# knowhunger/go-libp2p-pubsub

Hardware: AMD Instinct MI355X
Metric: peer-topic score updates/s + msg deliveries/s @1M peers, 1-8 GPUs, %HBM BW (higher is better)
Workload: dtype f64; 1 GPU; cfg3: 1M peers x 8 topics, full P1-P7 refreshScores()+score() per DecayInterval, connectSome d=6 overlay, spam-test topic params; peers_per_gpu=1000000, topics=8, pairs_per_gpu=11999954, records_per_gpu=95999632, parallelism=observers range-sharded, 1 shard(s), no exchange

## Files before the change

### go-libp2p-pubsub_amd/csrc/gsx_device.h

```cpp
#pragma once

#include <hip/hip_runtime.h>
#include <stdint.h>

namespace gsx {

struct DevTopicParams {
    double topic_weight;
    double w1, cap1;
    int64_t q1;
    double inv_q1;
    double w2, d2, cap2;
    double w3, d3, cap3, thr3;
    int64_t win3, act3;
    double w3b, d3b;
    double w4, d4;
    int32_t scored;
    int32_t pad;
};

__host__ __device__ __forceinline__ double q1_inverse(int64_t q1) { return q1 > 0 ? 1.0 / (double)q1 : 0.0; }

struct DevPeerParams {
    double topic_score_cap;
    double w5;
    double w6;
    int64_t thr6;
    double w7, thr7, d7;
    double decay_to_zero;
    int64_t retain_ns;
};

constexpr int KARG_TOPICS = 8;
struct KernParams {
    DevPeerParams pp;
    DevTopicParams tp[KARG_TOPICS];
};

constexpr int TILE = 64;
constexpr int NFIELD = 5;
enum Field { FMD = 0, MMD = 1, MFP = 2, IMD = 3, GRAFT = 4 };

__host__ __device__ __forceinline__ size_t rec_index(uint64_t p, uint32_t t, uint32_t n_topics, int field) {
    return (((p / TILE) * n_topics + t) * NFIELD + field) * TILE + (p % TILE);
}
__host__ __device__ __forceinline__ size_t flag_index(uint64_t p, uint32_t t, uint32_t n_topics) {
    return ((p / TILE) * n_topics + t) * TILE + (p % TILE);
}

constexpr uint8_t ZM_ZERO = 0, ZM_MAYBE = 1;
__host__ __device__ __forceinline__ size_t zmap_index(uint64_t p, uint32_t t, uint32_t n_topics, int field) {
    return ((p / TILE) * n_topics + t) * 2 + (size_t)(field - MFP);
}
__host__ __device__ __forceinline__ size_t zmap_bytes(uint64_t n_tiles, uint32_t n_topics) {
    return ((n_tiles * n_topics * 2 + 3) / 4 + 1) * 4;
}

constexpr int PZ_APP = 0, PZ_P6 = 1, PZ_ENTRY = 4;
__host__ __device__ __forceinline__ size_t pzmap_bytes(uint64_t n_tiles) { return (n_tiles + 1) * PZ_ENTRY; }

struct DevState {
    double* rec;
    uint8_t* rflags;
    uint8_t* zmap;
    uint8_t* pzmap;
    uint8_t* pflags;
    int64_t* expire;
    double* bp;
    double* app;
    const uint32_t* ipg;
    uint32_t* ipcount;
    double* score;
    const DevTopicParams* tp;
    uint64_t n_pairs;
    uint32_t n_topics;
    int64_t last_refresh;
    uint32_t phase;
    uint32_t wb_period;
    double decay_to_zero;
    double d7;
};

constexpr uint8_t REC_IN_MESH = 0x01;
constexpr uint8_t REC_ACTIVE = 0x02;
constexpr uint8_t REC_FRESH = 0x04;
constexpr uint8_t REC_EPOCH = 0x18;
constexpr int REC_EPOCH_SHIFT = 3;
constexpr uint8_t PAIR_PRESENT = 0x01;
constexpr uint8_t PAIR_CONNECTED = 0x02;
constexpr uint8_t PAIR_EPOCH = 0x0C;
constexpr int PAIR_EPOCH_SHIFT = 2;
constexpr uint32_t IPG_NONE = 0xFFFFFFFFu;
constexpr uint32_t IPG_WL = 0x80000000u;

struct DevEvent {
    uint32_t kind;
    uint32_t topic;
    uint64_t pair;
    int64_t now_ns;
    int64_t arg;
};

struct DevSynthSpec {
    uint64_t seed;
    int64_t now;
    double fmd_max, mmd_max, mfp_max, imd_max;
    double p_in_mesh;
    int64_t graft_window;
    double bp_max, p_disc, p_abs;
    int64_t expire_jitter;
    uint32_t sybil_first;
};

constexpr uint8_t EDGE_OUTBOUND = 0x01, EDGE_DIRECT = 0x02, EDGE_GOSSIPSUB = 0x04, EDGE_FLOODSUB = 0x08,
                  EDGE_NO_PX = 0x10;
constexpr uint32_t ROUTER_FLOODSUB = 0, ROUTER_GOSSIPSUB = 1, ROUTER_RANDOMSUB = 2;
constexpr uint32_t NO_PAIR = 0xFFFFFFFFu;
constexpr uint8_t FWD_FORWARD = 0x01;
constexpr uint8_t FWD_PUBLISH = 0x02;
constexpr uint8_t FWD_RSUB_CAND = 0x04;
constexpr uint8_t FWD_SEND = 0x07;
constexpr uint8_t FWD_GIN = 0x08;
constexpr int RANDOMSUB_D = 6;
// ... 814 lines not shown
```

### go-libp2p-pubsub_amd/csrc/gsx_engine.cpp

```cpp
#include <hip/hip_runtime.h>

#include <algorithm>
#include <map>
#include <atomic>
#include <chrono>
#include <array>
#include <cmath>
#include <cstdio>
#include <cstdlib>
#include <cstring>
#include <deque>
#include <functional>
#include <string>
#include <unordered_map>
#include <unordered_set>
#include <vector>

#include "../../include/gsx.h"
#include "gsx_device.h"

namespace {

constexpr int64_t kSecond = 1000000000LL;
constexpr int64_t kTimeCacheDuration = 120 * kSecond;
constexpr uint64_t kHostScoreMax = 1u << 16;

bool invalid_number(double x) { return std::isnan(x) || std::isinf(x); }

enum { kDeliveryUnknown = 0, kDeliveryValid, kDeliveryInvalid, kDeliveryIgnored, kDeliveryThrottled };

struct RecKey {
    uint32_t obs;
    uint64_t msg;
    bool operator==(const RecKey& o) const { return obs == o.obs && msg == o.msg; }
};
struct RecKeyHash {
    size_t operator()(const RecKey& k) const {
        uint64_t x = k.msg ^ (uint64_t(k.obs) * 0x9E3779B97F4A7C15ULL);
        x ^= x >> 31;
        x *= 0xbf58476d1ce4e5b9ULL;
        x ^= x >> 29;
        return size_t(x);
    }
};
struct DeliveryRecord {
    int status = kDeliveryUnknown;
    int64_t first_seen = 0;
    int64_t validated = 0;
    bool validated_set = false;
    std::vector<uint64_t> peers;
    bool peers_nil = false;
};

}

struct gsx_engine {
    int device = 0;
    hipStream_t stream = nullptr;
    hipEvent_t ev_start = nullptr, ev_stop = nullptr, ev_staged = nullptr;
    std::string err;

    uint32_t T = 0;
    gsx_peer_score_params pp{};
    bool pp_set = false;
    gsx_thresholds th{};
    gsx_topic_score_params tp[GSX_MAX_TOPICS]{};
    bool scored[GSX_MAX_TOPICS]{};
    gsx::DevTopicParams* d_tp = nullptr;

    bool loaded = false;
    uint32_t n_nodes = 0;
    uint64_t E = 0, rs = 0, n_tiles = 0;
    int64_t last_refresh = 0;
    uint32_t phase = 0;
    uint32_t wb_period = 4;
    bool retained_possible = false;
    int64_t retain_horizon = INT64_MIN;
    uint64_t purge_launches = 0;
    std::vector<int64_t> row_ptr;
    std::vector<int32_t> col_host;
    std::vector<uint32_t> pair_obs;
    std::vector<uint32_t> ipg_host;
    std::vector<uint32_t> group_ip;
    std::vector<uint8_t> ip_wl;
    uint32_t n_groups = 0;

    double* d_rec = nullptr;
    uint8_t* d_rflags = nullptr;
    uint8_t* d_zmap = nullptr;
    uint8_t* d_pzmap = nullptr;
    void* d_tmp = nullptr;
    uint32_t* d_nbad = nullptr;
    uint8_t *d_pflags = nullptr, *d_eflags = nullptr;
    int64_t* d_expire = nullptr;
    double *d_bp = nullptr, *d_app = nullptr, *d_score = nullptr;
    uint32_t *d_ipg = nullptr, *d_ipcount = nullptr;
    int32_t* d_col = nullptr;
    int64_t* d_row_ptr = nullptr;
    uint32_t* d_rev = nullptr;
    std::vector<uint8_t> eflags_host;
    bool floodsub_peers = true;
    int64_t max_deg = 0;

    gsx_gossipsub_params gp{};
    int64_t* d_backoff = nullptr;
    uint8_t* d_bo8 = nullptr;
    uint64_t *d_ctl = nullptr, *d_resp = nullptr;
    uint8_t* d_dirty = nullptr;
// ... 549 lines not shown
}

gsx::DevTopicParams dev_topic_params(const gsx_engine* e, uint32_t t);

gsx::KernParams kern_params(const gsx_engine* e) {
    gsx::KernParams k{};
    k.pp = dev_peer_params(e);
    for (uint32_t t = 0; t < e->T && t < (uint32_t)gsx::KARG_TOPICS; ++t) k.tp[t] = dev_topic_params(e, t);
    return k;
}

gsx::DevTopicParams dev_topic_params(const gsx_engine* e, uint32_t t) {
    gsx::DevTopicParams d{};
    const gsx_topic_score_params& p = e->tp[t];
    d.topic_weight = p.topic_weight;
    d.w1 = p.time_in_mesh_weight;
    d.cap1 = p.time_in_mesh_cap;
    d.q1 = e->scored[t] ? p.time_in_mesh_quantum_ns : 1;
    d.inv_q1 = gsx::q1_inverse(d.q1);
    d.w2 = p.first_message_deliveries_weight;
    d.d2 = p.first_message_deliveries_decay;
    d.cap2 = p.first_message_deliveries_cap;
    d.w3 = p.mesh_message_deliveries_weight;
    d.d3 = p.mesh_message_deliveries_decay;
    d.cap3 = p.mesh_message_deliveries_cap;
    d.thr3 = p.mesh_message_deliveries_threshold;
    d.win3 = p.mesh_message_deliveries_window_ns;
    d.act3 = p.mesh_message_deliveries_activation_ns;
    d.w3b = p.mesh_failure_penalty_weight;
    d.d3b = p.mesh_failure_penalty_decay;
    d.w4 = p.invalid_message_deliveries_weight;
    d.d4 = p.invalid_message_deliveries_decay;
    d.scored = e->scored[t] ? 1 : 0;
    return d;
}

int upload_topic_params(gsx_engine* e) {
    gsx::DevTopicParams h[GSX_MAX_TOPICS]{};
    for (uint32_t t = 0; t < e->T; ++t) h[t] = dev_topic_params(e, t);
    HIPCHK(e, hipMemcpyAsync(e->d_tp, h, sizeof(gsx::DevTopicParams) * GSX_MAX_TOPICS, hipMemcpyHostToDevice,
                             e->stream));
    HIPCHK(e, hipStreamSynchronize(e->stream));
    return GSX_OK;
}

void seen_release(gsx_engine* e, uint64_t* p, size_t ) {
    if (!p) return;
    auto it = e->seen_cap.find(p);
    e->seen_pool.emplace_back(it != e->seen_cap.end() ? it->second : 0, p);
}
uint64_t* seen_acquire(gsx_engine* e, size_t words) {
    size_t best = e->seen_pool.size();
    for (size_t i = 0; i < e->seen_pool.size(); ++i)
        if (e->seen_pool[i].first >= words && (best == e->seen_pool.size() || e->seen_pool[i].first < e->seen_pool[best].first))
            best = i;
    if (best < e->seen_pool.size()) {
        uint64_t* p = e->seen_pool[best].second;
        e->seen_pool.erase(e->seen_pool.begin() + (long)best);
        return p;
    }
    constexpr size_t kSlab = 4, kSlabMaxBytes = 64ull << 20;
    const size_t w = (std::max<size_t>(words, 1) + 31) & ~(size_t)31;
    const size_t n = 8 * w <= kSlabMaxBytes ? kSlab : 1;
    uint64_t* p = nullptr;
    if (hipMalloc((void**)&p, 8 * w * n) != hipSuccess) {
        if (n == 1 || hipMalloc((void**)&p, 8 * w) != hipSuccess) return nullptr;
// ... 1497 lines not shown
    return GSX_OK;
}

int gsx_refresh(gsx_engine* e, int64_t now) {
    if (!e) return GSX_EINVAL;
    if (!e->loaded) return fail(e, GSX_ESTATE, "no overlay loaded");
    if (int rc = fold_deferred(e)) return rc;
    int rc = flush(e);
    if (rc) return rc;
    const gsx::DevState s = dev_state(e);
    if (e->retained_possible) {
        HIPCHK(e, gsx::launch_purge(s, now, e->stream));
        ++e->purge_launches;
        if (now > e->retain_horizon) {
            e->retained_possible = false;
            e->retain_horizon = INT64_MIN;
        }
    }
    const bool region = e->t_active && e->t_used < e->t_max;
    HIPCHK(e, hipEventRecord(region ? e->tev[2 * e->t_used] : e->ev_start, e->stream));
    HIPCHK(e, rescore_all(e, s, now, true));
    HIPCHK(e, hipEventRecord(region ? e->tev[2 * e->t_used + 1] : e->ev_stop, e->stream));
    if (region) ++e->t_used;
    e->timed = !region;
    e->scores_exact();
    e->state_changed();
    e->last_refresh = now;
    e->phase = e->phase + 1 >= e->wb_period ? 0 : e->phase + 1;
    return GSX_OK;
}

int gsx_set_decay_writeback(gsx_engine* e, uint32_t k) {
    if (!e) return GSX_EINVAL;
    if (k != 1 && k != 2 && k != 4) return fail(e, GSX_EINVAL, "decay write-back period must be 1, 2 or 4");
    if (int rc = gx_busy(e)) return rc;
    if (int rc = fold_deferred(e)) return rc;
    if (int rc = flush(e)) return rc;
    if (int rc = materialize_all(e)) return rc;
    e->wb_period = k;
    return GSX_OK;
}

int gsx_last_refresh_ms(gsx_engine* e, float* ms) {
    if (!e || !ms) return GSX_EINVAL;
    if (!e->timed) return fail(e, GSX_ESTATE, "no refresh timed yet");
    HIPCHK(e, hipEventSynchronize(e->ev_stop));
    HIPCHK(e, hipEventElapsedTime(ms, e->ev_start, e->ev_stop));
    return GSX_OK;
}

int gsx_timing_begin(gsx_engine* e, uint32_t max_launches) {
    if (!e || max_launches == 0) return GSX_EINVAL;
    while (e->tev.size() < 2 * (size_t)max_launches) {
        hipEvent_t ev;
        HIPCHK(e, hipEventCreate(&ev));
        e->tev.push_back(ev);
    }
    e->t_max = max_launches;
    e->t_used = 0;
    e->t_active = true;
    return GSX_OK;
}

int gsx_timing_end(gsx_engine* e, double* total_ms, double* min_ms, double* max_ms, uint32_t* n) {
    if (!e || !total_ms || !n) return GSX_EINVAL;
    if (!e->t_active) return fail(e, GSX_ESTATE, "gsx_timing_begin not called");
    e->t_active = false;
    double sum = 0, lo = 0, hi = 0;
    for (uint32_t i = 0; i < e->t_used; ++i) {
        HIPCHK(e, hipEventSynchronize(e->tev[2 * i + 1]));
        float ms = 0;
        HIPCHK(e, hipEventElapsedTime(&ms, e->tev[2 * i], e->tev[2 * i + 1]));
// ... 5309 lines not shown
```

### go-libp2p-pubsub_amd/csrc/gsx_kernels.hip

```cpp
#include "gsx_ops.h"

namespace gsx {



template <int TT, bool REFRESH>
__global__ __launch_bounds__(256) void k_refresh_score(DevState s, KernParams kp, int64_t now,
                                                       const uint8_t* __restrict__ only,
                                                       const uint8_t* __restrict__ only2,
                                                       const unsigned long long* __restrict__ gate) {
    const uint64_t p = (uint64_t)blockIdx.x * 256u + threadIdx.x;
    if (p >= s.n_pairs) return;
    if (!REFRESH && gate && gate[0] + gate[1] == 0) return;
    if (!REFRESH && only && (!only[p] || (only2 && !only2[p]))) return;
    const int T = TT > 0 ? TT : (int)s.n_topics;
    const uint64_t lane = p % TILE;
    const uint64_t wtile = wave_uniform(p / TILE);
    const uint64_t zoff = wtile * (uint64_t)T * 2;
    uint32_t zm[TT > 0 ? TT : 1];
    if constexpr (TT > 0) {
#pragma unroll
        for (int t = 0; t < TT; ++t) zm[t] = zmap_pair(s.zmap, zoff + 2 * t);
    }
    const uint32_t pz = __builtin_amdgcn_readfirstlane(reinterpret_cast<const uint32_t*>(s.pzmap)[wtile]);
    const bool app_maybe = (pz >> (8 * PZ_APP)) & 0xFFu;
    const bool p6_maybe = !REFRESH || ((pz >> (8 * PZ_P6)) & 0xFFu);
    const uint8_t st = s.pflags[p];
    if (!(st & PAIR_PRESENT)) {
        s.score[p] = 0.0;
        return;
    }
    const DevPeerParams& pp = kp.pp;
    double p5 = 0.0;
    if (app_maybe) p5 = s.app[p];
    const bool conn = REFRESH && (st & PAIR_CONNECTED);
    const uint32_t phase = s.phase;
    const bool wb = REFRESH && phase + 1 >= s.wb_period;
    const bool lag = st & PAIR_CONNECTED;
    const uint8_t keep_conn = (uint8_t)~(REC_FRESH | (wb ? REC_EPOCH : 0));
    double* const tile = s.rec + (p / TILE) * (uint64_t)T * (NFIELD * TILE) + lane;
    uint8_t* const ftile = s.rflags + (p / TILE) * (uint64_t)T * TILE + lane;
    double score = 0.0;
    auto topic_step = [&](int t, const DevTopicParams& tp, double fmd, double mmd, double mfp, double imd,
                          int64_t graft, uint8_t fl, uint32_t zmt) {
        double* const r = tile + (uint64_t)t * (NFIELD * TILE);
        const double fmd0 = fmd, mmd0 = mmd, mfp0 = mfp, imd0 = imd;
        const uint32_t nd = (lag ? (phase - ((uint32_t)fl >> REC_EPOCH_SHIFT)) & 3u : 0u) + (conn ? 1u : 0u);
        const uint32_t nd0 = __builtin_amdgcn_readfirstlane(nd);
        auto decay_all = [&]() {
            fmd = decay(fmd, tp.d2, pp.decay_to_zero);
            mmd = decay(mmd, tp.d3, pp.decay_to_zero);
            mfp = decay(mfp, tp.d3b, pp.decay_to_zero);
            imd = decay(imd, tp.d4, pp.decay_to_zero);
        };
        if (__ballot(nd != nd0) == 0) {
            for (uint32_t i = 0; i < nd0; ++i) decay_all();
        } else {
            for (uint32_t i = 0; i < nd; ++i) decay_all();
        }
        if (wb) {
            if (conn && __double_as_longlong(fmd) != __double_as_longlong(fmd0)) __builtin_nontemporal_store(fmd, r + FMD * TILE);
            if (conn && __double_as_longlong(mmd) != __double_as_longlong(mmd0)) __builtin_nontemporal_store(mmd, r + MMD * TILE);
            if (conn && __double_as_longlong(mfp) != __double_as_longlong(mfp0)) __builtin_nontemporal_store(mfp, r + MFP * TILE);
            if (conn && __double_as_longlong(imd) != __double_as_longlong(imd0)) __builtin_nontemporal_store(imd, r + IMD * TILE);
        }
        const bool in_mesh = fl & REC_IN_MESH;
        int64_t mt = 0;
        if (conn) {
            mt = in_mesh ? now - graft : 0;
            const uint8_t nf = (uint8_t)((fl & keep_conn) | ((in_mesh && mt > tp.act3) ? REC_ACTIVE : 0));
            if (nf != fl) ftile[t * TILE] = nf;
            fl = nf;
        } else if (in_mesh && !(fl & REC_FRESH)) {
            mt = s.last_refresh - graft;
        }
        if constexpr (REFRESH) {
            if (zmt && __ballot(1) == ~0ull) {
                uint8_t* const zb = s.zmap + zoff + 2 * t;
                const bool z3 = (zmt & ZM_MFP_BITS) && __ballot(__double_as_longlong(mfp) != 0) == 0;
                const bool z4 = (zmt & ZM_IMD_BITS) && __ballot(__double_as_longlong(imd) != 0) == 0;
                if (z3 && !wb && __double_as_longlong(mfp0) != 0) r[MFP * TILE] = 0.0;
                if (z4 && !wb && __double_as_longlong(imd0) != 0) r[IMD * TILE] = 0.0;
                if (z3 && lane == 0) zb[0] = ZM_ZERO;
                if (z4 && lane == 0) zb[1] = ZM_ZERO;
            }
        }
        score += topic_score(tp, fl, mt, fmd, mmd, mfp, imd);
    };
    if constexpr (TT > 0) {
        double fmd[TT], mmd[TT], mfp[TT], imd[TT];
        int64_t gr[TT];
// ... 2 lines not shown
        for (int t = 0; t < TT; ++t) {
            if (!kp.tp[t].scored) continue;
            const double* const r = tile + (uint64_t)t * (NFIELD * TILE);
            fmd[t] = __builtin_nontemporal_load(r + FMD * TILE);
            mmd[t] = __builtin_nontemporal_load(r + MMD * TILE);
            mfp[t] = (zm[t] & ZM_MFP_BITS) ? __builtin_nontemporal_load(r + MFP * TILE) : 0.0;
            imd[t] = (zm[t] & ZM_IMD_BITS) ? __builtin_nontemporal_load(r + IMD * TILE) : 0.0;
            fl[t] = ftile[t * TILE];
            gr[t] = (TT > 1 || (fl[t] & REC_IN_MESH))
                        ? __builtin_nontemporal_load(reinterpret_cast<const int64_t*>(r) + GRAFT * TILE)
                        : 0;
        }
#pragma unroll
        for (int t = 0; t < TT; ++t) {
            if (!kp.tp[t].scored) continue;
            topic_step(t, kp.tp[t], fmd[t], mmd[t], mfp[t], imd[t], gr[t], fl[t], zm[t]);
        }
    } else {
        for (int t = 0; t < T; ++t) {
            const DevTopicParams& tp = s.tp[t];
            if (!tp.scored) continue;
            const double* const r = tile + (uint64_t)t * (NFIELD * TILE);
            const uint32_t zmt = zmap_pair(s.zmap, zoff + 2 * t);
            const uint8_t fl = ftile[t * TILE];
            const int64_t graft = (fl & REC_IN_MESH) ? reinterpret_cast<const int64_t*>(r)[GRAFT * TILE] : 0;
            const double fmd = __builtin_nontemporal_load(r + FMD * TILE), mmd = __builtin_nontemporal_load(r + MMD * TILE);
            const double mfp = (zmt & ZM_MFP_BITS) ? __builtin_nontemporal_load(r + MFP * TILE) : 0.0;
            const double imd = (zmt & ZM_IMD_BITS) ? __builtin_nontemporal_load(r + IMD * TILE) : 0.0;
            topic_step(t, tp, fmd, mmd, mfp, imd, graft, fl, zmt);
        }
    }
    const double bp0 = s.bp[p];
    double bp = bp0;
    const uint32_t nb = (lag ? (phase - ((uint32_t)st >> PAIR_EPOCH_SHIFT)) & 3u : 0u) + (conn ? 1u : 0u);
    const uint32_t nb0 = __builtin_amdgcn_readfirstlane(nb);
    if (__ballot(nb != nb0) == 0) {
        for (uint32_t i = 0; i < nb0; ++i) bp = decay(bp, pp.d7, pp.decay_to_zero);
    } else {
        for (uint32_t i = 0; i < nb; ++i) bp = decay(bp, pp.d7, pp.decay_to_zero);
    }
    if (wb && conn) {
        if (__double_as_longlong(bp) != __double_as_longlong(bp0)) s.bp[p] = bp;
        if (st & PAIR_EPOCH) s.pflags[p] = st & ~PAIR_EPOCH;
    }
    double p6 = 0.0;
    const bool p6_read = pp.w6 != 0.0 && p6_maybe;
    if (p6_read) p6 = ip_colocation(s, pp, p);
    s.score[p] = score_tail_vals(pp, score, p5, p6, bp);
    if constexpr (REFRESH) {
        if ((app_maybe || p6_read) && __ballot(1) == ~0ull) {
            uint8_t* const pzb = s.pzmap + wtile * PZ_ENTRY;
            const bool z5 = app_maybe && __ballot(__double_as_longlong(p5) != 0) == 0;
            const bool z6 = p6_read && __ballot(__double_as_longlong(p6) != 0) == 0;
            if (z5 && lane == 0) pzb[PZ_APP] = ZM_ZERO;
            if (z6 && lane == 0) pzb[PZ_P6] = ZM_ZERO;
        }
    }
}

__global__ __launch_bounds__(256) void k_purge(DevState s, int64_t now) {
    const uint64_t p = (uint64_t)blockIdx.x * 256u + threadIdx.x;
    if (p >= s.n_pairs) return;
    const uint8_t st = s.pflags[p];
    if ((st & (PAIR_PRESENT | PAIR_CONNECTED)) != PAIR_PRESENT) return;
    if (!(now > s.expire[p])) return;
    s.pflags[p] = 0;
    const uint2 g = reinterpret_cast<const uint2*>(s.ipg)[p];
    if (g.x != IPG_NONE) atomicSub(&s.ipcount[g.x & ~IPG_WL], 1u);
    if (g.y != IPG_NONE && g.y != g.x) atomicSub(&s.ipcount[g.y & ~IPG_WL], 1u);
}
// ... 459 lines not shown
```

### go-libp2p-pubsub_amd/csrc/gsx_ops.h

```cpp
#pragma once

#include "gsx_device.h"

namespace gsx {


__device__ __forceinline__ double ip_colocation(const DevState& s, const DevPeerParams& pp, uint64_t p) {
    const uint2 g = reinterpret_cast<const uint2*>(s.ipg)[p];
    double result = 0.0;
    const uint32_t gs[2] = {g.x, g.y};
#pragma unroll
    for (int k = 0; k < 2; ++k) {
        const uint32_t id = gs[k];
        if (id == IPG_NONE || (id & IPG_WL)) continue;
        const int64_t peers_in_ip = (int64_t)s.ipcount[id];
        if (peers_in_ip > pp.thr6) {
            const double surpluss = (double)(peers_in_ip - pp.thr6);
            result += surpluss * surpluss;
        }
    }
    return result;
}

template <class F>
// ... 104 lines not shown
    x *= d;
    return x < dtz ? 0.0 : x;
}

__device__ __forceinline__ void zmap_mark(const DevState& s, uint64_t p, uint32_t t, int field) {
    s.zmap[zmap_index(p, t, s.n_topics, field)] = ZM_MAYBE;
}

__device__ __forceinline__ uint64_t wave_uniform(uint64_t x) {
    return (uint64_t)__builtin_amdgcn_readfirstlane((uint32_t)x) |
           (uint64_t)__builtin_amdgcn_readfirstlane((uint32_t)(x >> 32)) << 32;
}

constexpr uint32_t ZM_MFP_BITS = 0x00FFu, ZM_IMD_BITS = 0xFF00u;
__device__ __forceinline__ uint32_t zmap_pair(const uint8_t* zmap, uint64_t o) {
    const uint32_t w = reinterpret_cast<const uint32_t*>(zmap)[o >> 2];
    return __builtin_amdgcn_readfirstlane((w >> ((uint32_t)(o & 2) * 8)) & 0xFFFFu);
}

__device__ __forceinline__ void pzmap_mark(const DevState& s, uint64_t p, int which) {
    s.pzmap[(p / TILE) * PZ_ENTRY + which] = ZM_MAYBE;
}
__device__ __forceinline__ void pzmap_mark_row(const DevState& s, uint64_t lo, uint64_t hi) {
    if (hi > s.n_pairs) hi = s.n_pairs;
    if (lo >= hi) return;
    for (uint64_t tile = lo / TILE; tile <= (hi - 1) / TILE; ++tile) s.pzmap[tile * PZ_ENTRY + PZ_P6] = ZM_MAYBE;
}

struct RecVals {
    double fmd, mmd, mfp, imd;
};

__device__ __forceinline__ uint32_t rec_pend(const DevState& s, uint8_t st, uint8_t fl, const DevTopicParams& tp) {
    return ((st & PAIR_CONNECTED) && tp.scored) ? ((s.phase - ((uint32_t)fl >> REC_EPOCH_SHIFT)) & 3u) : 0u;
}

__device__ __forceinline__ void rec_decay(RecVals& v, const DevTopicParams& tp, double dtz, uint32_t k) {
    for (uint32_t i = 0; i < k; ++i) {
        v.fmd = decay(v.fmd, tp.d2, dtz);
        v.mmd = decay(v.mmd, tp.d3, dtz);
        v.mfp = decay(v.mfp, tp.d3b, dtz);
        v.imd = decay(v.imd, tp.d4, dtz);
    }
}

__device__ __forceinline__ RecVals rec_read(const DevState& s, uint64_t p, uint32_t t, uint8_t st, uint8_t fl) {
    const size_t b = rec_index(p, t, s.n_topics, FMD);
    RecVals v = {s.rec[b + FMD * TILE], s.rec[b + MMD * TILE], s.rec[b + MFP * TILE], s.rec[b + IMD * TILE]};
    rec_decay(v, s.tp[t], s.decay_to_zero, rec_pend(s, st, fl, s.tp[t]));
    return v;
}
__device__ __forceinline__ RecVals rec_read(const DevState& s, uint64_t p, uint32_t t) {
    return rec_read(s, p, t, s.pflags[p], s.rflags[flag_index(p, t, s.n_topics)]);
}

__device__ __forceinline__ void rec_store_decayed(const DevState& s, uint64_t p, uint32_t t, uint32_t k) {
    const size_t b = rec_index(p, t, s.n_topics, FMD);
    const RecVals o = {s.rec[b + FMD * TILE], s.rec[b + MMD * TILE], s.rec[b + MFP * TILE], s.rec[b + IMD * TILE]};
    RecVals v = o;
    rec_decay(v, s.tp[t], s.decay_to_zero, k);
    if (__double_as_longlong(v.fmd) != __double_as_longlong(o.fmd)) s.rec[b + FMD * TILE] = v.fmd;
    if (__double_as_longlong(v.mmd) != __double_as_longlong(o.mmd)) s.rec[b + MMD * TILE] = v.mmd;
    if (__double_as_longlong(v.mfp) != __double_as_longlong(o.mfp)) {
        if (__double_as_longlong(v.mfp) != 0) zmap_mark(s, p, t, MFP);
        s.rec[b + MFP * TILE] = v.mfp;
    }
    if (__double_as_longlong(v.imd) != __double_as_longlong(o.imd)) {
        if (__double_as_longlong(v.imd) != 0) zmap_mark(s, p, t, IMD);
        s.rec[b + IMD * TILE] = v.imd;
    }
}

__device__ __forceinline__ uint8_t rec_materialize(const DevState& s, uint64_t p, uint32_t t, uint8_t st) {
    const size_t fi = flag_index(p, t, s.n_topics);
    const uint8_t fl = s.rflags[fi];
    const uint32_t k = rec_pend(s, st, fl, s.tp[t]);
    if (k) rec_store_decayed(s, p, t, k);
    const uint8_t nf = (uint8_t)((fl & ~REC_EPOCH) | (s.phase << REC_EPOCH_SHIFT));
    if (nf != fl) s.rflags[fi] = nf;
    return nf;
}
__device__ __forceinline__ uint8_t rec_materialize(const DevState& s, uint64_t p, uint32_t t) {
    return rec_materialize(s, p, t, s.pflags[p]);
}

__device__ __forceinline__ uint32_t bp_pend(const DevState& s, uint8_t st) {
    return (st & PAIR_CONNECTED) ? ((s.phase - ((uint32_t)st >> PAIR_EPOCH_SHIFT)) & 3u) : 0u;
}

__device__ __forceinline__ double bp_decay(double bp, double d7, double dtz, uint32_t k) {
    for (uint32_t i = 0; i < k; ++i) bp = decay(bp, d7, dtz);
    return bp;
}

__device__ __forceinline__ double bp_read(const DevState& s, uint64_t p, uint8_t st) {
    return bp_decay(s.bp[p], s.d7, s.decay_to_zero, bp_pend(s, st));
}

__device__ __forceinline__ uint8_t bp_materialize(const DevState& s, uint64_t p, uint8_t st) {
    if (!(st & PAIR_CONNECTED)) return st;
    const uint32_t k = bp_pend(s, st);
    if (k) {
        const double o = s.bp[p], v = bp_decay(o, s.d7, s.decay_to_zero, k);
        if (__double_as_longlong(v) != __double_as_longlong(o)) s.bp[p] = v;
    }
    const uint8_t nf = (uint8_t)((st & ~PAIR_EPOCH) | ((s.phase & 3u) << PAIR_EPOCH_SHIFT));
    if (nf != st) s.pflags[p] = nf;
    return nf;
}

__device__ __forceinline__ double eval_pair(const DevState& s, const DevPeerParams& pp, uint64_t p) {
    const uint8_t st = s.pflags[p];
    if (!(st & PAIR_PRESENT)) return 0.0;
    double score = 0.0;
    for (uint32_t t = 0; t < s.n_topics; ++t) {
        const DevTopicParams& tp = s.tp[t];
        if (!tp.scored) continue;
        const uint8_t fl = s.rflags[flag_index(p, t, s.n_topics)];
        const RecVals v = rec_read(s, p, t, st, fl);
        score += topic_score(tp, fl, mesh_time_of(s, fl, p, t), v.fmd, v.mmd, v.mfp, v.imd);
    }
    return score_tail(s, pp, p, score, bp_read(s, p, st));
}

__device__ __forceinline__ double add_ones_capped(double x, uint32_t k, double cap) {
    while (k && !(x >= 1.0 && x < 4503599627370496.0)) {
        x = x + 1;
        --k;
        if (x > cap) return cap;
    }
    while (k) {
        const unsigned long long bits = (unsigned long long)__double_as_longlong(x);
        const double top = __longlong_as_double((long long)((((bits >> 52) & 0x7FF) + 1) << 52));
        const double gap = top - x;
        const double s = ceil(gap) - 1;
        if (s >= (double)k) {
            x = x + (double)k;
            k = 0;
        } else {
            x = x + s;
            k -= (uint32_t)s;
            x = x + 1;
            --k;
        }
        if (x > cap) return cap;
        if (!(x < 4503599627370496.0))
            while (k) {
                x = x + 1;
                --k;
                if (x > cap) return cap;
            }
    }
    return x > cap ? cap : x;
}


__device__ __forceinline__ void ipcount_add(const DevState& s, uint64_t p, int delta) {
    const uint2 g = reinterpret_cast<const uint2*>(s.ipg)[p];
    if (g.x != IPG_NONE) s.ipcount[g.x & ~IPG_WL] += (uint32_t)delta;
    if (g.y != IPG_NONE && g.y != g.x) s.ipcount[g.y & ~IPG_WL] += (uint32_t)delta;
}

__device__ __forceinline__ bool scored_topic(const DevState& s, uint64_t p, uint32_t topic) {
    return (s.pflags[p] & PAIR_PRESENT) && topic < s.n_topics && s.tp[topic].scored;
}

__device__ inline void ev_add_peer(const DevState& s, const DevPeerParams& pp, uint64_t p, uint64_t row_lo,
                                   uint64_t row_hi) {
    const uint8_t st = s.pflags[p];
    const uint8_t ep = (uint8_t)(s.phase << REC_EPOCH_SHIFT);
    if (!(st & PAIR_PRESENT)) {
        for (uint32_t t = 0; t < s.n_topics; ++t) {
            const size_t b = rec_index(p, t, s.n_topics, FMD);
            for (int f = 0; f < NFIELD; ++f) s.rec[b + f * TILE] = 0.0;
            s.rflags[flag_index(p, t, s.n_topics)] = ep;
        }
        s.bp[p] = 0.0;
        s.expire[p] = 0;
        ipcount_add(s, p, +1);
        const uint2 g = reinterpret_cast<const uint2*>(s.ipg)[p];
        const bool over_x = g.x != IPG_NONE && !(g.x & IPG_WL) && (int64_t)s.ipcount[g.x] > pp.thr6;
        const bool over_y = g.y != IPG_NONE && !(g.y & IPG_WL) && (int64_t)s.ipcount[g.y] > pp.thr6;
        if (over_x || over_y) {
            pzmap_mark(s, p, PZ_P6);
            pzmap_mark_row(s, row_lo, row_hi);
        }
    } else if (!(st & PAIR_CONNECTED)) {
        for (uint32_t t = 0; t < s.n_topics; ++t) {
            const size_t fi = flag_index(p, t, s.n_topics);
            const uint8_t fl = s.rflags[fi];
            if ((fl & REC_EPOCH) != ep) s.rflags[fi] = (uint8_t)((fl & ~REC_EPOCH) | ep);
        }
    }
    if (!(st & PAIR_PRESENT) || !(st & PAIR_CONNECTED))
        s.pflags[p] = (uint8_t)(PAIR_PRESENT | PAIR_CONNECTED | ((s.phase & 3u) << PAIR_EPOCH_SHIFT));
}

__device__ inline void ev_remove_peer(const DevState& s, const DevPeerParams& pp, uint64_t p, int64_t now) {
    const uint8_t st = s.pflags[p];
    if (!(st & PAIR_PRESENT)) return;
    if (eval_pair(s, pp, p) > 0) {
        ipcount_add(s, p, -1);
        bp_materialize(s, p, st);
        s.pflags[p] = 0;
        return;
    }
    for (uint32_t t = 0; t < s.n_topics; ++t) {
        const DevTopicParams& tp = s.tp[t];
        if (!tp.scored) continue;
        const size_t b = rec_index(p, t, s.n_topics, FMD);
        const size_t fi = flag_index(p, t, s.n_topics);
        const uint8_t fl = rec_materialize(s, p, t, st);
        s.rec[b + FMD * TILE] = 0.0;
        const double threshold = tp.thr3;
        const double mmd = s.rec[b + MMD * TILE];
        if ((fl & REC_IN_MESH) && (fl & REC_ACTIVE) && mmd < threshold) {
            const double deficit = threshold - mmd;
            zmap_mark(s, p, t, MFP);
            s.rec[b + MFP * TILE] = s.rec[b + MFP * TILE] + deficit * deficit;
        }
        s.rflags[fi] = fl & ~(REC_IN_MESH | REC_FRESH);
    }
    bp_materialize(s, p, st);
    s.pflags[p] = PAIR_PRESENT;
    s.expire[p] = now + pp.retain_ns;
}

__device__ inline void ev_graft(const DevState& s, uint64_t p, uint32_t topic, int64_t now) {
// ... 124 lines not shown
```

### go-libp2p-pubsub_amd/gsx/abi.py

```python
from __future__ import annotations

import ctypes as C
import os

HERE = os.path.dirname(os.path.abspath(__file__))
LIB_PATH = os.environ.get("GSX_LIB") or os.path.join(HERE, "libgsx.so")

GSX_OK = 0
GSX_EINVAL = -22
GSX_ENOMEM = -12
GSX_ENODEV = -19
GSX_ERANGE = -34
GSX_ESTATE = -71
GSX_EDEVICE = -5

GSX_MAX_TOPICS = 64
GSX_NO_IP = 0xFFFFFFFF

GSX_EDGE_OUTBOUND = 0x01
GSX_EDGE_DIRECT = 0x02
GSX_EDGE_GOSSIPSUB = 0x04
GSX_EDGE_FLOODSUB = 0x08
GSX_EDGE_NO_PX = 0x10

# ... 590 lines not shown
    "gsx_refresh": (C.c_int, [C.c_void_p, C.c_int64]),
    "gsx_scores": (C.c_int, [C.c_void_p, P(C.c_double), C.c_size_t]),
    "gsx_score": (C.c_int, [C.c_void_p, C.c_uint64, P(C.c_double)]),
    "gsx_score_many": (C.c_int, [C.c_void_p, P(C.c_uint64), C.c_size_t, P(C.c_double)]),
    "gsx_gx_pending": (C.c_int, [C.c_void_p, P(C.c_uint32)]),
    "gsx_gx_common": (C.c_int, [C.c_void_p, P(C.c_uint64)]),
    "gsx_gx_set_common": (C.c_int, [C.c_void_p, P(C.c_uint64)]),
    "gsx_gx_pack_ihave": (C.c_int, [C.c_void_p, C.c_void_p]),
    "gsx_gx_recv_ihave": (C.c_int, [C.c_void_p, C.c_void_p]),
    "gsx_gx_rows_words": (C.c_int, [C.c_void_p, P(C.c_uint32)]),
    "gsx_gx_rows_pack": (C.c_int, [C.c_void_p, P(C.c_uint64), C.c_void_p]),
    "gsx_gx_rows_recv": (C.c_int, [C.c_void_p, C.c_void_p, C.c_uint64]),
    "gsx_gx_exchange": (C.c_int, [C.c_void_p, P(C.c_uint32)]),
    "gsx_gxf_begin": (C.c_int, [C.c_void_p, C.c_uint32]),
    "gsx_gxf_entry_words": (C.c_int, [C.c_void_p, P(C.c_uint32)]),
    "gsx_gxf_pack_fout": (C.c_int, [C.c_void_p, C.c_void_p]),
    "gsx_gxf_recv_fout": (C.c_int, [C.c_void_p, C.c_void_p]),
    "gsx_gxf_pack": (C.c_int, [C.c_void_p, C.c_uint32, P(C.c_uint64), C.c_void_p]),
    "gsx_gxf_step": (C.c_int, [C.c_void_p, C.c_uint32, C.c_void_p, C.c_uint64, P(C.c_uint64)]),
    "gsx_gxf_pack_dev": (C.c_int, [C.c_void_p, C.c_uint32, C.c_void_p, C.c_void_p]),
    "gsx_gxf_end": (C.c_int, [C.c_void_p]),
    "gsx_gx_got": (C.c_int, [C.c_void_p, P(C.c_uint8)]),
    "gsx_gx_end": (C.c_int, [C.c_void_p, P(C.c_uint8), P(HeartbeatOut)]),
    "gsx_device_scores": (C.c_int, [C.c_void_p, P(C.c_void_p)]),
    "gsx_sync": (C.c_int, [C.c_void_p]),
    "gsx_settle_scores": (C.c_int, [C.c_void_p]),
    "gsx_import_state": (C.c_int, [C.c_void_p, P(StateView)]),
    "gsx_export_state": (C.c_int, [C.c_void_p, P(StateView)]),
    "gsx_zero_map_violations": (C.c_int, [C.c_void_p, P(C.c_uint64)]),
    "gsx_zero_map_marked": (C.c_int, [C.c_void_p, P(C.c_uint64)]),
    "gsx_pair_zero_map_violations": (C.c_int, [C.c_void_p, P(C.c_uint64)]),
    "gsx_pair_zero_map_marked": (C.c_int, [C.c_void_p, C.c_uint32, P(C.c_uint64)]),
    "gsx_set_decay_writeback": (C.c_int, [C.c_void_p, C.c_uint32]),
    "gsx_purge_launches": (C.c_int, [C.c_void_p, P(C.c_uint64)]),
    "gsx_last_refresh_ms": (C.c_int, [C.c_void_p, P(C.c_float)]),
    "gsx_synthesize_state": (C.c_int, [C.c_void_p, P(SynthSpec)]),
    "gsx_propagate": (C.c_int, [C.c_void_p, C.c_void_p, C.c_size_t, P(PropConfig), P(PropOut)]),
    "gsx_prop_results": (C.c_int, [C.c_void_p, P(C.c_uint8), P(C.c_int32)]),
    "gsx_prop_stats": (C.c_int, [C.c_void_p, C.c_void_p, C.c_void_p, C.c_void_p]),
    "gsx_set_link_latency": (C.c_int, [C.c_void_p, P(C.c_uint8), C.c_size_t]),
    "gsx_propagate_timed": (C.c_int, [C.c_void_p, C.c_void_p, C.c_size_t, P(PropConfig), C.c_uint32, P(TimedOut)]),
    "gsx_timed_results": (C.c_int, [C.c_void_p, P(C.c_uint16), P(C.c_int32)]),
    "gsx_timed_stats": (C.c_int, [C.c_void_p, C.c_uint32, C.c_uint32, C.c_void_p, C.c_void_p, C.c_void_p]),
    "gsx_timed_traffic": (C.c_int, [C.c_void_p, C.c_void_p, C.c_uint32, C.c_uint32, P(TimedTrafficOut)]),
    "gsx_score_stats_edges": (C.c_int, [C.c_void_p, P(ScoreStatsSpec)]),
    "gsx_score_stats": (C.c_int, [C.c_void_p, P(ScoreStatsSpec), P(ScoreStatsOut)]),
    "gsx_score_parts": (C.c_int, [C.c_void_p, P(ScoreStatsSpec), P(ScorePartsOut)]),
    "gsx_mesh_stats": (C.c_int, [C.c_void_p, P(MeshStatsSpec), P(MeshStatsOut)]),
    "gsx_prop_set_tracking": (C.c_int, [C.c_void_p, C.c_uint32]),
    "gsx_prop_duplicates": (C.c_int, [C.c_void_p, P(C.c_uint64), C.c_size_t]),
    "gsx_prop_traffic": (C.c_int, [C.c_void_p, C.c_void_p, C.c_void_p, C.c_void_p, C.c_void_p, C.c_void_p,
                                   C.c_void_p]),
    "gsx_set_pair_ips": (C.c_int, [C.c_void_p, P(C.c_uint64), P(C.c_uint32), C.c_size_t]),
    "gsx_peer_score_snapshot": (C.c_int, [C.c_void_p, P(ScoreSnapshot)]),
    "gsx_prop_pending_invalid": (C.c_int, [C.c_void_p, C.c_void_p]),
    "gsx_prop_replace_pending_invalid": (C.c_int, [C.c_void_p, C.c_void_p]),
    "gsx_prop_pending_credits": (C.c_int, [C.c_void_p, C.c_void_p, C.c_void_p]),
    "gsx_prop_fold_credits": (C.c_int, [C.c_void_p, C.c_void_p, C.c_void_p]),
    "gsx_set_stream": (C.c_int, [C.c_void_p, C.c_void_p]),
    "gsx_load_overlay_shard": (
        C.c_int,
        [C.c_void_p, C.c_uint32, C.c_uint32, C.c_uint32, P(C.c_int64), P(C.c_int32), P(C.c_uint8), P(C.c_uint32)],
    ),
    "gsx_shard_recv_plan": (C.c_int, [C.c_void_p, C.c_uint32, P(C.c_uint32), _u64p, P(C.c_uint32), P(C.c_uint32)]),
    "gsx_shard_send_plan": (C.c_int, [C.c_void_p, _u64p, P(C.c_uint32), P(C.c_uint32)]),
    "gsx_shard_counts": (C.c_int, [C.c_void_p, _u64p, _u64p]),
# ... 115 lines not shown
```

### go-libp2p-pubsub_amd/gsx/engine.py

```python
from __future__ import annotations

import ctypes as C
from typing import Dict, Iterable, Optional

import numpy as np

from . import abi
from .abi import GsxError, prop_words


def _ptr(a: Optional[np.ndarray], ctype):
    if a is None:
        return C.cast(None, C.POINTER(ctype))
    return a.ctypes.data_as(C.POINTER(ctype))


_CTYPES = {"<f8": C.c_double, "<i8": C.c_int64, "u1": C.c_uint8}


def default_gossipsub_params(**kw) -> abi.GossipSubParams:
    gp = abi.GossipSubParams()
    rc = abi.load_library().gsx_default_gossipsub_params(C.byref(gp))
    if rc != 0:
        raise RuntimeError(f"gsx_default_gossipsub_params -> {rc}")
# ... 1435 lines not shown
        self._chk(self.lib.gsx_synthesize_state(self.h, C.byref(spec)), "gsx_synthesize_state")

    def snapshot(self) -> Dict[str, np.ndarray]:
        out = {f: np.empty(self.n_pairs, dtype=d) for f, d in abi.SNAPSHOT_PAIR.items()}
        out.update({f: np.empty(self.n_topics * self.n_pairs, dtype=d) for f, d in abi.SNAPSHOT_RECORD.items()})
        sv = abi.ScoreSnapshot(**{f: out[f].ctypes.data_as(dict(abi.ScoreSnapshot._fields_)[f]) for f in out})
        self._chk(self.lib.gsx_peer_score_snapshot(self.h, C.byref(sv)), "gsx_peer_score_snapshot")
        return out

    def export_state(self) -> Dict[str, np.ndarray]:
        R = self.n_topics * self.n_pairs
        out = {}
        for f in abi.STATE_FIELDS:
            n = R if f in abi.RECORD_FIELDS else self.n_pairs
            out[f] = np.empty(n, dtype=abi.STATE_DTYPES[f])
        sv = self._view(out)
        self._chk(self.lib.gsx_export_state(self.h, C.byref(sv)), "gsx_export_state")
        out["last_refresh_ns"] = int(sv.last_refresh_ns)
        return out

    def zero_map_violations(self) -> int:
        n = C.c_uint64()
        self._chk(self.lib.gsx_zero_map_violations(self.h, C.byref(n)), "gsx_zero_map_violations")
        return n.value

    def set_decay_writeback(self, k: int) -> None:
        self._chk(self.lib.gsx_set_decay_writeback(self.h, k), "gsx_set_decay_writeback")

    def zero_map_marked(self) -> int:
        n = C.c_uint64()
        self._chk(self.lib.gsx_zero_map_marked(self.h, C.byref(n)), "gsx_zero_map_marked")
        return n.value

    def pair_zero_map_violations(self) -> int:
        n = C.c_uint64()
        self._chk(self.lib.gsx_pair_zero_map_violations(self.h, C.byref(n)), "gsx_pair_zero_map_violations")
        return n.value

    def pair_zero_map_marked(self, which: int) -> int:
        n = C.c_uint64()
        self._chk(self.lib.gsx_pair_zero_map_marked(self.h, which, C.byref(n)), "gsx_pair_zero_map_marked")
        return n.value

    def purge_launches(self) -> int:
        n = C.c_uint64()
        self._chk(self.lib.gsx_purge_launches(self.h, C.byref(n)), "gsx_purge_launches")
        return n.value
```

### include/gsx.h

```cpp
#ifndef GSX_H
#define GSX_H

#include <stddef.h>
#include <stdint.h>

#ifdef __cplusplus
extern "C" {
#endif

#define GSX_ABI_VERSION 5

#define GSX_OK 0
#define GSX_EINVAL (-22)
#define GSX_ENOMEM (-12)
#define GSX_ENODEV (-19)
#define GSX_ERANGE (-34)
#define GSX_ESTATE (-71)
#define GSX_EDEVICE (-5)


typedef struct gsx_topic_score_params {
    double topic_weight;
    double time_in_mesh_weight;
    int64_t time_in_mesh_quantum_ns;
// ... 230 lines not shown
typedef struct gsx_mesh_stats_spec {
    int64_t now_ns;
    uint32_t n_bins;
    uint32_t n_age_edges;
    int64_t age_edges_ns[GSX_MS_MAX_AGE_EDGES];
    const uint8_t* node_class;
    uint32_t n_classes;
    uint32_t hostile_mask;
    uint32_t min_honest;
    uint32_t symmetry;
} gsx_mesh_stats_spec;

typedef struct gsx_mesh_stats_out {
    uint64_t* topic_tot;
    uint64_t* deg_hist;
    uint64_t* out_hist;
    uint64_t* in_hist;
    uint64_t* age_hist;
    uint64_t* class_links;
    uint32_t* node_deg;
    uint32_t* node_out;
    uint32_t* node_in;
    uint32_t* node_class_deg;
} gsx_mesh_stats_out;
int gsx_mesh_stats(gsx_engine* e, const gsx_mesh_stats_spec* spec, const gsx_mesh_stats_out* out);

int gsx_zero_map_violations(gsx_engine* e, uint64_t* n);
int gsx_zero_map_marked(gsx_engine* e, uint64_t* n);
int gsx_pair_zero_map_violations(gsx_engine* e, uint64_t* n);
#define GSX_PZ_APP 0u
#define GSX_PZ_P6 1u
int gsx_pair_zero_map_marked(gsx_engine* e, uint32_t which, uint64_t* n);
int gsx_set_decay_writeback(gsx_engine* e, uint32_t k);
int gsx_purge_launches(gsx_engine* e, uint64_t* n);

typedef struct gsx_score_snapshot {
    uint8_t* present;
    double* score;
    double* app_specific_score;
    double* ip_colocation_factor;
    double* behaviour_penalty;
    int64_t* time_in_mesh_ns;
    double* first_message_deliveries;
    double* mesh_message_deliveries;
    double* invalid_message_deliveries;
} gsx_score_snapshot;
int gsx_peer_score_snapshot(gsx_engine* e, gsx_score_snapshot* s);

typedef struct gsx_synth_spec {
    uint64_t seed;
    int64_t now_ns;
    double fmd_max, mmd_max, mfp_max, imd_max_sybil;
    double p_in_mesh;
    int64_t graft_window_ns;
    double bp_max;
    double p_disconnected, p_absent;
    int64_t expire_jitter_ns;
    uint32_t sybil_first_node;
    uint32_t reserved;
} gsx_synth_spec;

int gsx_synthesize_state(gsx_engine* e, const gsx_synth_spec* spec);

int gsx_last_refresh_ms(gsx_engine* e, float* ms);

enum gsx_router { GSX_ROUTER_FLOODSUB = 0, GSX_ROUTER_GOSSIPSUB = 1, GSX_ROUTER_RANDOMSUB = 2 };
// ... 362 lines not shown
```

Measured before the change: 136.6 billion peer-topic score updates/s.

## Widen decay epoch to 4 bits and default write-back period to 16

Widens the record and pair epoch fields from 2 to 4 bits so decayed counters can be written back to HBM only every 16 refreshes instead of every 4, making 16 the default. This cuts per-refresh store traffic on the large record array. It also replaces the per-step decay-to-zero test with repeated multiplication followed by one threshold test, which is valid when every decay factor lies in (0,1). The cost is a longer multiply chain for lagging records, more flag bits per byte, and a new getter API.

```diff
diff --git a/go-libp2p-pubsub_amd/csrc/gsx_device.h b/go-libp2p-pubsub_amd/csrc/gsx_device.h
--- a/go-libp2p-pubsub_amd/csrc/gsx_device.h
+++ b/go-libp2p-pubsub_amd/csrc/gsx_device.h
@@ -16,8 +16,10 @@
     double w3b, d3b;
     double w4, d4;
     int32_t scored;
-    int32_t pad;
-};
+    int32_t chain;
+};
+
+__host__ __device__ __forceinline__ bool decay_chain_ok(double d) { return d > 0.0 && d < 1.0; }
 
 __host__ __device__ __forceinline__ double q1_inverse(int64_t q1) { return q1 > 0 ? 1.0 / (double)q1 : 0.0; }
 
@@ -84,11 +86,12 @@
 constexpr uint8_t REC_IN_MESH = 0x01;
 constexpr uint8_t REC_ACTIVE = 0x02;
 constexpr uint8_t REC_FRESH = 0x04;
-constexpr uint8_t REC_EPOCH = 0x18;
+constexpr uint32_t EPOCH_MASK = 15u;
+constexpr uint8_t REC_EPOCH = 0x78;
 constexpr int REC_EPOCH_SHIFT = 3;
 constexpr uint8_t PAIR_PRESENT = 0x01;
 constexpr uint8_t PAIR_CONNECTED = 0x02;
-constexpr uint8_t PAIR_EPOCH = 0x0C;
+constexpr uint8_t PAIR_EPOCH = 0x3C;
 constexpr int PAIR_EPOCH_SHIFT = 2;
 constexpr uint32_t IPG_NONE = 0xFFFFFFFFu;
 constexpr uint32_t IPG_WL = 0x80000000u;
diff --git a/go-libp2p-pubsub_amd/csrc/gsx_engine.cpp b/go-libp2p-pubsub_amd/csrc/gsx_engine.cpp
--- a/go-libp2p-pubsub_amd/csrc/gsx_engine.cpp
+++ b/go-libp2p-pubsub_amd/csrc/gsx_engine.cpp
@@ -54,6 +54,13 @@
 
 }
 
+#ifndef GSX_WB_PERIOD_DEFAULT
+#define GSX_WB_PERIOD_DEFAULT 16
+#endif
+static_assert(GSX_WB_PERIOD_DEFAULT == 1 || GSX_WB_PERIOD_DEFAULT == 2 || GSX_WB_PERIOD_DEFAULT == 4 ||
+                  GSX_WB_PERIOD_DEFAULT == 16,
+              "the periods gsx_set_decay_writeback accepts");
+
 struct gsx_engine {
     int device = 0;
     hipStream_t stream = nullptr;
@@ -73,7 +80,7 @@
     uint64_t E = 0, rs = 0, n_tiles = 0;
     int64_t last_refresh = 0;
     uint32_t phase = 0;
-    uint32_t wb_period = 4;
+    uint32_t wb_period = GSX_WB_PERIOD_DEFAULT;
     bool retained_possible = false;
     int64_t retain_horizon = INT64_MIN;
     uint64_t purge_launches = 0;
@@ -689,6 +696,10 @@
     d.w4 = p.invalid_message_deliveries_weight;
     d.d4 = p.invalid_message_deliveries_decay;
     d.scored = e->scored[t] ? 1 : 0;
+    d.chain = gsx::decay_chain_ok(d.d2) && gsx::decay_chain_ok(d.d3) && gsx::decay_chain_ok(d.d3b) &&
+                      gsx::decay_chain_ok(d.d4)
+                  ? 1
+                  : 0;
     return d;
 }
 
@@ -2252,12 +2263,19 @@
 
 int gsx_set_decay_writeback(gsx_engine* e, uint32_t k) {
     if (!e) return GSX_EINVAL;
-    if (k != 1 && k != 2 && k != 4) return fail(e, GSX_EINVAL, "decay write-back period must be 1, 2 or 4");
+    if (k != 1 && k != 2 && k != 4 && k != 16)
+        return fail(e, GSX_EINVAL, "decay write-back period must be 1, 2, 4 or 16");
     if (int rc = gx_busy(e)) return rc;
     if (int rc = fold_deferred(e)) return rc;
     if (int rc = flush(e)) return rc;
     if (int rc = materialize_all(e)) return rc;
     e->wb_period = k;
+    return GSX_OK;
+}
+
+int gsx_get_decay_writeback(gsx_engine* e, uint32_t* k) {
+    if (!e || !k) return GSX_EINVAL;
+    *k = e->wb_period;
     return GSX_OK;
 }
 
diff --git a/go-libp2p-pubsub_amd/csrc/gsx_kernels.hip b/go-libp2p-pubsub_amd/csrc/gsx_kernels.hip
--- a/go-libp2p-pubsub_amd/csrc/gsx_kernels.hip
+++ b/go-libp2p-pubsub_amd/csrc/gsx_kernels.hip
@@ -38,6 +38,7 @@
     const bool wb = REFRESH && phase + 1 >= s.wb_period;
     const bool lag = st & PAIR_CONNECTED;
     const uint8_t keep_conn = (uint8_t)~(REC_FRESH | (wb ? REC_EPOCH : 0));
+    const bool chain_dtz = pp.decay_to_zero > 0.0;
     double* const tile = s.rec + (p / TILE) * (uint64_t)T * (NFIELD * TILE) + lane;
     uint8_t* const ftile = s.rflags + (p / TILE) * (uint64_t)T * TILE + lane;
     double score = 0.0;
@@ -45,18 +46,35 @@
                           int64_t graft, uint8_t fl, uint32_t zmt) {
         double* const r = tile + (uint64_t)t * (NFIELD * TILE);
         const double fmd0 = fmd, mmd0 = mmd, mfp0 = mfp, imd0 = imd;
-        const uint32_t nd = (lag ? (phase - ((uint32_t)fl >> REC_EPOCH_SHIFT)) & 3u : 0u) + (conn ? 1u : 0u);
+        const uint32_t nd = (lag ? (phase - ((uint32_t)fl >> REC_EPOCH_SHIFT)) & EPOCH_MASK : 0u) + (conn ? 1u : 0u);
         const uint32_t nd0 = __builtin_amdgcn_readfirstlane(nd);
-        auto decay_all = [&]() {
-            fmd = decay(fmd, tp.d2, pp.decay_to_zero);
-            mmd = decay(mmd, tp.d3, pp.decay_to_zero);
-            mfp = decay(mfp, tp.d3b, pp.decay_to_zero);
-            imd = decay(imd, tp.d4, pp.decay_to_zero);
+        auto mul_all = [&]() {
+            fmd *= tp.d2;
+            mmd *= tp.d3;
+            mfp *= tp.d3b;
+            imd *= tp.d4;
         };
-        if (__ballot(nd != nd0) == 0) {
-            for (uint32_t i = 0; i < nd0; ++i) decay_all();
+        auto test_all = [&](bool any) {
+            fmd = (any && fmd < pp.decay_to_zero) ? 0.0 : fmd;
+            mmd = (any && mmd < pp.decay_to_zero) ? 0.0 : mmd;
+            mfp = (any && mfp < pp.decay_to_zero) ? 0.0 : mfp;
+            imd = (any && imd < pp.decay_to_zero) ? 0.0 : imd;
+        };
+        if (tp.chain && chain_dtz) {
+            if (__ballot(nd != nd0) == 0) {
+#pragma clang loop unroll(disable)
+                for (uint32_t i = 0; i < nd0; ++i) mul_all();
+                if (nd0) test_all(true);
+            } else {
+#pragma clang loop unroll(disable)
+                for (uint32_t i = 0; i < nd; ++i) mul_all();
+                test_all(nd != 0);
+            }
         } else {
-            for (uint32_t i = 0; i < nd; ++i) decay_all();
+            for (uint32_t i = 0; i < nd; ++i) {
+                mul_all();
+                test_all(true);
+            }
         }
         if (wb) {
             if (conn && __double_as_longlong(fmd) != __double_as_longlong(fmd0)) __builtin_nontemporal_store(fmd, r + FMD * TILE);
@@ -125,10 +143,18 @@
     }
     const double bp0 = s.bp[p];
     double bp = bp0;
-    const uint32_t nb = (lag ? (phase - ((uint32_t)st >> PAIR_EPOCH_SHIFT)) & 3u : 0u) + (conn ? 1u : 0u);
+    const uint32_t nb = (lag ? (phase - ((uint32_t)st >> PAIR_EPOCH_SHIFT)) & EPOCH_MASK : 0u) + (conn ? 1u : 0u);
     const uint32_t nb0 = __builtin_amdgcn_readfirstlane(nb);
-    if (__ballot(nb != nb0) == 0) {
-        for (uint32_t i = 0; i < nb0; ++i) bp = decay(bp, pp.d7, pp.decay_to_zero);
+    if (decay_chain_ok(pp.d7) && chain_dtz) {
+        if (__ballot(nb != nb0) == 0) {
+#pragma clang loop unroll(disable)
+            for (uint32_t i = 0; i < nb0; ++i) bp *= pp.d7;
+            if (nb0) bp = bp < pp.decay_to_zero ? 0.0 : bp;
+        } else {
+#pragma clang loop unroll(disable)
+            for (uint32_t i = 0; i < nb; ++i) bp *= pp.d7;
+            bp = (nb && bp < pp.decay_to_zero) ? 0.0 : bp;
+        }
     } else {
         for (uint32_t i = 0; i < nb; ++i) bp = decay(bp, pp.d7, pp.decay_to_zero);
     }
diff --git a/go-libp2p-pubsub_amd/csrc/gsx_ops.h b/go-libp2p-pubsub_amd/csrc/gsx_ops.h
--- a/go-libp2p-pubsub_amd/csrc/gsx_ops.h
+++ b/go-libp2p-pubsub_amd/csrc/gsx_ops.h
@@ -160,10 +160,30 @@
 };
 
 __device__ __forceinline__ uint32_t rec_pend(const DevState& s, uint8_t st, uint8_t fl, const DevTopicParams& tp) {
-    return ((st & PAIR_CONNECTED) && tp.scored) ? ((s.phase - ((uint32_t)fl >> REC_EPOCH_SHIFT)) & 3u) : 0u;
+    return ((st & PAIR_CONNECTED) && tp.scored) ? ((s.phase - ((uint32_t)fl >> REC_EPOCH_SHIFT)) & EPOCH_MASK) : 0u;
+}
+
+__device__ __forceinline__ double decay_chain(double x, double d, double dtz, uint32_t k) {
+    for (uint32_t i = 0; i < k; ++i) x *= d;
+    return (k && x < dtz) ? 0.0 : x;
 }
 
 __device__ __forceinline__ void rec_decay(RecVals& v, const DevTopicParams& tp, double dtz, uint32_t k) {
+    if (tp.chain && dtz > 0.0) {
+        for (uint32_t i = 0; i < k; ++i) {
+            v.fmd *= tp.d2;
+            v.mmd *= tp.d3;
+            v.mfp *= tp.d3b;
+            v.imd *= tp.d4;
+        }
+        if (k) {
+            v.fmd = v.fmd < dtz ? 0.0 : v.fmd;
+            v.mmd = v.mmd < dtz ? 0.0 : v.mmd;
+            v.mfp = v.mfp < dtz ? 0.0 : v.mfp;
+            v.imd = v.imd < dtz ? 0.0 : v.imd;
+        }
+        return;
+    }
     for (uint32_t i = 0; i < k; ++i) {
         v.fmd = decay(v.fmd, tp.d2, dtz);
         v.mmd = decay(v.mmd, tp.d3, dtz);
@@ -204,7 +224,7 @@
     const uint8_t fl = s.rflags[fi];
     const uint32_t k = rec_pend(s, st, fl, s.tp[t]);
     if (k) rec_store_decayed(s, p, t, k);
-    const uint8_t nf = (uint8_t)((fl & ~REC_EPOCH) | (s.phase << REC_EPOCH_SHIFT));
+    const uint8_t nf = (uint8_t)((fl & ~REC_EPOCH) | ((s.phase & EPOCH_MASK) << REC_EPOCH_SHIFT));
     if (nf != fl) s.rflags[fi] = nf;
     return nf;
 }
@@ -213,10 +233,11 @@
 }
 
 __device__ __forceinline__ uint32_t bp_pend(const DevState& s, uint8_t st) {
-    return (st & PAIR_CONNECTED) ? ((s.phase - ((uint32_t)st >> PAIR_EPOCH_SHIFT)) & 3u) : 0u;
+    return (st & PAIR_CONNECTED) ? ((s.phase - ((uint32_t)st >> PAIR_EPOCH_SHIFT)) & EPOCH_MASK) : 0u;
 }
 
 __device__ __forceinline__ double bp_decay(double bp, double d7, double dtz, uint32_t k) {
+    if (decay_chain_ok(d7) && dtz > 0.0) return decay_chain(bp, d7, dtz, k);
     for (uint32_t i = 0; i < k; ++i) bp = decay(bp, d7, dtz);
     return bp;
 }
@@ -232,7 +253,7 @@
         const double o = s.bp[p], v = bp_decay(o, s.d7, s.decay_to_zero, k);
         if (__double_as_longlong(v) != __double_as_longlong(o)) s.bp[p] = v;
     }
-    const uint8_t nf = (uint8_t)((st & ~PAIR_EPOCH) | ((s.phase & 3u) << PAIR_EPOCH_SHIFT));
+    const uint8_t nf = (uint8_t)((st & ~PAIR_EPOCH) | ((s.phase & EPOCH_MASK) << PAIR_EPOCH_SHIFT));
     if (nf != st) s.pflags[p] = nf;
     return nf;
 }
@@ -296,7 +317,7 @@
 __device__ inline void ev_add_peer(const DevState& s, const DevPeerParams& pp, uint64_t p, uint64_t row_lo,
                                    uint64_t row_hi) {
     const uint8_t st = s.pflags[p];
-    const uint8_t ep = (uint8_t)(s.phase << REC_EPOCH_SHIFT);
+    const uint8_t ep = (uint8_t)((s.phase & EPOCH_MASK) << REC_EPOCH_SHIFT);
     if (!(st & PAIR_PRESENT)) {
         for (uint32_t t = 0; t < s.n_topics; ++t) {
             const size_t b = rec_index(p, t, s.n_topics, FMD);
@@ -321,7 +342,7 @@
         }
     }
     if (!(st & PAIR_PRESENT) || !(st & PAIR_CONNECTED))
-        s.pflags[p] = (uint8_t)(PAIR_PRESENT | PAIR_CONNECTED | ((s.phase & 3u) << PAIR_EPOCH_SHIFT));
+        s.pflags[p] = (uint8_t)(PAIR_PRESENT | PAIR_CONNECTED | ((s.phase & EPOCH_MASK) << PAIR_EPOCH_SHIFT));
 }
 
 __device__ inline void ev_remove_peer(const DevState& s, const DevPeerParams& pp, uint64_t p, int64_t now) {
diff --git a/go-libp2p-pubsub_amd/gsx/abi.py b/go-libp2p-pubsub_amd/gsx/abi.py
--- a/go-libp2p-pubsub_amd/gsx/abi.py
+++ b/go-libp2p-pubsub_amd/gsx/abi.py
@@ -646,6 +646,7 @@
     "gsx_pair_zero_map_violations": (C.c_int, [C.c_void_p, P(C.c_uint64)]),
     "gsx_pair_zero_map_marked": (C.c_int, [C.c_void_p, C.c_uint32, P(C.c_uint64)]),
     "gsx_set_decay_writeback": (C.c_int, [C.c_void_p, C.c_uint32]),
+    "gsx_get_decay_writeback": (C.c_int, [C.c_void_p, P(C.c_uint32)]),
     "gsx_purge_launches": (C.c_int, [C.c_void_p, P(C.c_uint64)]),
     "gsx_last_refresh_ms": (C.c_int, [C.c_void_p, P(C.c_float)]),
     "gsx_synthesize_state": (C.c_int, [C.c_void_p, P(SynthSpec)]),
diff --git a/go-libp2p-pubsub_amd/gsx/engine.py b/go-libp2p-pubsub_amd/gsx/engine.py
--- a/go-libp2p-pubsub_amd/gsx/engine.py
+++ b/go-libp2p-pubsub_amd/gsx/engine.py
@@ -1491,6 +1491,11 @@
         self._chk(self.lib.gsx_zero_map_marked(self.h, C.byref(n)), "gsx_zero_map_marked")
         return n.value
 
+    def decay_writeback(self) -> int:
+        k = C.c_uint32()
+        self._chk(self.lib.gsx_get_decay_writeback(self.h, C.byref(k)), "gsx_get_decay_writeback")
+        return k.value
+
     def pair_zero_map_violations(self) -> int:
         n = C.c_uint64()
         self._chk(self.lib.gsx_pair_zero_map_violations(self.h, C.byref(n)), "gsx_pair_zero_map_violations")
diff --git a/include/gsx.h b/include/gsx.h
--- a/include/gsx.h
+++ b/include/gsx.h
@@ -286,6 +286,7 @@
 #define GSX_PZ_P6 1u
 int gsx_pair_zero_map_marked(gsx_engine* e, uint32_t which, uint64_t* n);
 int gsx_set_decay_writeback(gsx_engine* e, uint32_t k);
+int gsx_get_decay_writeback(gsx_engine* e, uint32_t* k);
 int gsx_purge_launches(gsx_engine* e, uint64_t* n);
 
 typedef struct gsx_score_snapshot {
```

After: 142.9 billion peer-topic score updates/s (median of 6 runs). 4.6% higher.
